# PeterFWS/Structure-PLP-SLAM

Hardware: AMD Instinct MI355X
Metric: frames/sec ORB+LSD extract+match, 640x480 TUM-RGBD, 1/2/4/8 GPU (higher is better)
Workload: dtype u8

## Files before the change

### structure-plp-slam_amd/csrc/line_kernels.hip

```cpp
#include <hip/hip_runtime.h>
#include <stdint.h>

#include <algorithm>
#include <cstdlib>

#include "blur_tile.hpp"
#include "plp_barrier.hpp"
#include "line_device.hpp"
#include "plp_common.hpp"
#include "sincos_ziv.hpp"
#include "xcd_map.hpp"

namespace plp {

struct TileDiv { uint32_t gx_magic, tiles_x_magic; };
static inline TileDiv tile_div(int tiles, int tiles_x, int B) { return TileDiv{plp_div_magic((uint32_t)tiles, (uint64_t)tiles * B), plp_div_magic((uint32_t)tiles_x, (uint64_t)tiles)}; }

__device__ __forceinline__ int reflect101_l(int p, int len) {
    if (len == 1) return 0;
    while (p < 0 || p >= len) p = p < 0 ? -p : 2 * (len - 1) - p;
    return p;
}

__device__ __forceinline__ float fast_atan2_deg_l(float y, float x) {
    const float p1 = 0.9997878412794807f * (float)(180 / 3.14159265358979323846);
    const float p3 = -0.3258083974640975f * (float)(180 / 3.14159265358979323846);
    const float p5 = 0.1555786518463281f * (float)(180 / 3.14159265358979323846);
    const float p7 = -0.04432655554792128f * (float)(180 / 3.14159265358979323846);
    const float eps = (float)2.2204460492503131e-16;
    const float ax = fabsf(x), ay = fabsf(y);
    float a;
    if (ax >= ay) {
        const float c = __fdiv_rn(ay, __fadd_rn(ax, eps));
        const float c2 = __fmul_rn(c, c);
        a = __fmul_rn(__fadd_rn(__fmul_rn(__fadd_rn(__fmul_rn(__fadd_rn(__fmul_rn(p7, c2), p5), c2), p3), c2), p1), c);
    } else {
        const float c = __fdiv_rn(ax, __fadd_rn(ay, eps));
        const float c2 = __fmul_rn(c, c);
        a = __fsub_rn(90.f, __fmul_rn(__fadd_rn(__fmul_rn(__fadd_rn(__fmul_rn(__fadd_rn(__fmul_rn(p7, c2), p5), c2), p3), c2), p1), c));
    }
    if (x < 0) a = __fsub_rn(180.f, a);
    if (y < 0) a = __fsub_rn(360.f, a);
    return a;
}

template <int R>
__global__ __launch_bounds__(256) __attribute__((amdgpu_waves_per_eu(8, 8))) void k_blur_plane(const uint8_t* __restrict__ src, size_t src_fs, int src_pitch,
                                                    uint8_t* __restrict__ dst, size_t dst_fs, int dst_pitch, int w, int h, BlurTapsN taps, TileDiv td) {
    __shared__ BlurTileLds<R> S;
    const int tiles_x = (w + kBlurTW - 1) / kBlurTW;
    unsigned t, f;
    xcd_frame_major(t, f, td.gx_magic);
    const int trow = (int)plp_div(t, (unsigned)tiles_x, td.tiles_x_magic);
    blur_tile<R>(S, src + (size_t)f * src_fs, src_pitch, dst + (size_t)f * dst_fs, dst_pitch, w, h,
                 ((int)t - trow * tiles_x) * kBlurTW, trow * kBlurTH, taps.k);
}

__global__ __launch_bounds__(256) void k_resize_exact(const uint8_t* __restrict__ src, size_t src_fs, int src_pitch,
                                                      uint8_t* __restrict__ dst, size_t dst_fs, int dst_pitch, int dw, int dh,
                                                      ResizeExactTab t) {
    const int dy = blockIdx.y * 4 + threadIdx.y, dx0 = (blockIdx.x * 64 + threadIdx.x) * 4;
    if (dy >= dh || dx0 >= dw) return;
    const uint8_t* s = src + (size_t)blockIdx.z * src_fs;
    const int yo = t.yo[dy], yc = t.yc[dy];
    const uint8_t* S0 = s + (size_t)yo * src_pitch;
    const uint8_t* S1 = yc < 0 ? S0 : S0 + src_pitch;
    const uint32_t b1 = yc < 0 ? 0u : (uint32_t)yc, b0 = 256u - b1;
    uint32_t packed = 0;
#pragma unroll
    for (int i = 0; i < 4; ++i) {
        const int dx = min(dx0 + i, dw - 1);
        const int xo = t.xo[dx], xc = t.xc[dx];
        uint32_t h0, h1;
        if (xc < 0) { h0 = (uint32_t)S0[xo] * 256u; h1 = (uint32_t)S1[xo] * 256u; }
        else {
            h0 = (uint32_t)S0[xo] * (uint32_t)(256 - xc) + (uint32_t)S0[xo + 1] * (uint32_t)xc;
            h1 = (uint32_t)S1[xo] * (uint32_t)(256 - xc) + (uint32_t)S1[xo + 1] * (uint32_t)xc;
        }
        const uint32_t v = (b0 * h0 + b1 * h1 + 32768u) >> 16;
        packed |= min(v, 255u) << (8 * i);
    }
    *reinterpret_cast<uint32_t*>(dst + (size_t)blockIdx.z * dst_fs + (size_t)dy * dst_pitch + dx0) = packed;
}

__global__ __launch_bounds__(256) __attribute__((amdgpu_waves_per_eu(8, 8))) void k_blur_half(const uint8_t* __restrict__ src, size_t src_fs, int src_pitch,
                                                                                           uint8_t* __restrict__ dst, size_t dst_fs, int dst_pitch, int w, int h, BlurTapsN taps, TileDiv td) {
    __shared__ BlurTileLds<5> S;
    const int tiles_x = (w + kBlurTW - 1) / kBlurTW;
    unsigned t, f;
    xcd_frame_major(t, f, td.gx_magic);
    const int trow = (int)plp_div(t, (unsigned)tiles_x, td.tiles_x_magic);
    const int tx0 = ((int)t - trow * tiles_x) * kBlurTW, ty0 = trow * kBlurTH;
    uint8_t* d = dst + (size_t)f * dst_fs;
    blur_tile_core<5>(S, src + (size_t)f * src_fs, src_pitch, w, h, tx0, ty0, taps.k, [&](int r0, int c4, const uint32_t (&rows)[kBlurRS]) {
        const int x = tx0 + c4;
        if (x >= w) return;
#pragma unroll
        for (int j = 0; j < 2; ++j) {
            const int y = ty0 + r0 + 2 * j;
            if (y >= h) continue;
            const uint32_t lo = __builtin_amdgcn_udot4(rows[2 * j], 0x00000101u, __builtin_amdgcn_udot4(rows[2 * j + 1], 0x00000101u, 2u, false), false) >> 2;
            const uint32_t hi = __builtin_amdgcn_udot4(rows[2 * j], 0x01010000u, __builtin_amdgcn_udot4(rows[2 * j + 1], 0x01010000u, 2u, false), false) >> 2;
            *reinterpret_cast<uint16_t*>(d + (size_t)(y >> 1) * dst_pitch + (x >> 1)) = (uint16_t)(lo | (hi << 8));
        }
    });
}

__global__ __launch_bounds__(256) void k_lsd_gradient(LinePlanes P, LsdParams lp) {
    __shared__ uint32_t s_list[256];
    __shared__ uint32_t s_max[4], s_cnt[4];
    const int b = blockIdx.y, tid = threadIdx.x, lane = tid & 63, wv = tid >> 6;
    const int idx = blockIdx.x * 256 + tid;
    const int n = P.sw * P.sh;
    uint32_t g2_def = 0, g2_any = 0, packed = 0;
    if (idx < n) {
        const int y = P.sw_magic ? (int)__umulhi((uint32_t)idx, P.sw_magic) : idx / P.sw, x = idx - y * P.sw;
        if (x < P.sw - 1 && y < P.sh - 1) {
            const uint8_t* s = P.scaled + ((size_t)b * P.sh + y) * P.spitch + x;
            const int DA = (int)s[P.spitch + 1] - (int)s[0];
            const int BC = (int)s[1] - (int)s[P.spitch];
            const int gx = DA + BC, gy = DA - BC;
            const uint32_t g2 = (uint32_t)(gx * gx + gy * gy);
            g2_any = g2;
            if (g2 >= lp.g2_def_min) {
                g2_def = g2;
                packed = (uint32_t)tid | ((uint32_t)(gx + 512) << 8) | ((uint32_t)(gy + 512) << 18);
            }
        }
        P.g2[(size_t)b * n + idx] = lp.seed_exact ? g2_any : g2_def;
    }
    const unsigned long long undef = __ballot(g2_def == 0);
    if (lane == 0 && blockIdx.x * 256 + tid < ((n + 63) / 64) * 64) P.undef[(size_t)b * ((n + 63) / 64) + (blockIdx.x * 256 + tid) / 64] = undef;
    const unsigned long long defm = ~undef;
    const int rank = __popcll(defm & ((1ull << lane) - 1ull));
    uint32_t mx = g2_def;
#pragma unroll
    for (int o = 32; o > 0; o >>= 1) mx = max(mx, (uint32_t)__shfl_xor((int)mx, o));
    if (lane == 0) { s_max[wv] = mx; s_cnt[wv] = (uint32_t)__popcll(defm); }
    wg_barrier();
    const uint32_t c0 = s_cnt[0], c1 = s_cnt[1], c2 = s_cnt[2], c3 = s_cnt[3];
    const int base = (wv > 0 ? (int)c0 : 0) + (wv > 1 ? (int)c1 : 0) + (wv > 2 ? (int)c2 : 0);
    if (g2_def) s_list[base + rank] = packed;
    if (tid == 0) P.blockmax[(size_t)b * gridDim.x + blockIdx.x] = max(max(s_max[0], s_max[1]), max(s_max[2], s_max[3]));
    wg_barrier();
    const int total = (int)(c0 + c1 + c2 + c3);
    if (tid < total) {
        const uint32_t e = s_list[tid];
        const int gx = (int)((e >> 8) & 1023u) - 512, gy = (int)(e >> 18) - 512;
        LsdPix px;
        px.deg = fast_atan2_deg_l((float)gx, (float)-gy);
        px.g2 = (uint32_t)(gx * gx + gy * gy);
        const float fa = (float)((double)px.deg * (3.14159265358979323846 / 180));
        if (!sincos_ziv(fa, &px.cs.x, &px.cs.y)) px.cs = make_float2((float)cos((double)fa), (float)sin((double)fa));
        P.pix[(size_t)b * n + blockIdx.x * 256 + (int)(e & 255u)] = px;
    }
}

__global__ __launch_bounds__(256) void k_lsd_order(LinePlanes P, LsdParams lp, int n_grad_blocks) {
    __shared__ uint32_t cnt[4][1024];
    __shared__ uint32_t s_red[4], s_wsum[4];
    const int b = blockIdx.x, tid = threadIdx.x, lane = tid & 63, q = tid >> 6;
    const int n = P.sw * P.sh, nv = (P.sw - 1) * (P.sh - 1);
    uint32_t mx = 0;
    for (int i = tid; i < n_grad_blocks; i += 256) mx = max(mx, P.blockmax[(size_t)b * n_grad_blocks + i]);
#pragma unroll
    for (int o = 32; o > 0; o >>= 1) mx = max(mx, (uint32_t)__shfl_xor((int)mx, o));
    if (lane == 0) s_red[q] = mx;
    for (int i = tid; i < 4096; i += 256) (&cnt[0][0])[i] = 0;
    wg_barrier();
    mx = max(max(s_red[0], s_red[1]), max(s_red[2], s_red[3]));
    const double max_grad = sqrt((double)mx / 4.0);
    const double bin_coef = (max_grad > 0) ? (double)(lp.n_bins - 1) / max_grad : 0;
    const uint32_t* g2 = P.g2 + (size_t)b * n;
    uint32_t* order = P.order + (size_t)b * nv;
    const int ngroups = (n + 63) / 64, gper = (ngroups + 3) / 4, g0 = q * gper, g1 = min(ngroups, g0 + gper);
    uint32_t* comp = P.reg + (size_t)b * P.reg_frame_stride + (size_t)g0 * 64;
    int ncomp = 0;
    for (int gb = g0; gb < g1; gb += 4) {
        uint32_t v4[4];
#pragma unroll
        for (int u = 0; u < 4; ++u) {
            const int pix = (gb + u) * 64 + lane;
            v4[u] = (gb + u < g1 && pix < n) ? g2[pix] : 0u;
        }
#pragma unroll
        for (int u = 0; u < 4; ++u) {
            const uint32_t v = v4[u];
            const unsigned long long defm = __ballot(v != 0);
            if (!defm) continue;
            if (v) {
                const uint32_t bin = (uint32_t)(int)(sqrt((double)v / 4.0) * bin_coef);
                atomicAdd(&cnt[q][bin], 1u);
                comp[ncomp + __popcll(defm & ((1ull << lane) - 1ull))] = (uint32_t)((gb + u) * 64 + lane) | (bin << kLsdSeedPixBits);
            }
            ncomp += __popcll(defm);
        }
    }
    wg_barrier();
    {
        const int v0 = 1023 - 4 * tid;
        uint32_t c[4][4], tot = 0;
#pragma unroll
        for (int j = 0; j < 4; ++j)
#pragma unroll
            for (int k = 0; k < 4; ++k) { c[j][k] = cnt[k][v0 - j]; tot += c[j][k]; }
        uint32_t inc = tot;
#pragma unroll
        for (int o = 1; o < 64; o <<= 1) { const uint32_t t = (uint32_t)__shfl_up((int)inc, o); if (lane >= o) inc += t; }
        if (lane == 63) s_wsum[q] = inc;
        wg_barrier();
        uint32_t run = inc - tot;
        for (int k = 0; k < q; ++k) run += s_wsum[k];
#pragma unroll
        for (int j = 0; j < 4; ++j)
#pragma unroll
            for (int k = 0; k < 4; ++k) { cnt[k][v0 - j] = run; run += c[j][k]; }
        if (tid == 255) P.n_order[b] = (int32_t)run;
    }
    wg_barrier();
    for (int ib = 0; ib < ncomp; ib += 256) {
    uint32_t e4[4];
#pragma unroll
    for (int u = 0; u < 4; ++u) e4[u] = ib + 64 * u + lane < ncomp ? comp[ib + 64 * u + lane] : 0u;
#pragma unroll
    for (int u = 0; u < 4; ++u) {
        const int i0 = ib + 64 * u;
        if (i0 >= ncomp) break;
        const bool valid = i0 + lane < ncomp;
        const uint32_t e = e4[u];
        const unsigned v = e >> kLsdSeedPixBits;
        unsigned long long peers = __ballot(valid);
#pragma unroll
        for (int bit = 0; bit < 10; ++bit) {
            const unsigned long long m = __ballot((v >> bit) & 1u);
            peers &= ((v >> bit) & 1u) ? m : ~m;
        }
        if (valid) {
// ... 1078 lines not shown
                if (tot <= kMwInline) {
                    if (lane < acc_n) e->inl[lane] = heap_ld(g.reg + lane);
                    else if (lane < tot) e->inl[lane] = g.assumed[lane - acc_n];
                }
                __builtin_amdgcn_fence(__ATOMIC_RELEASE, PLP_MW_SCOPE_NAME);
                __builtin_amdgcn_wave_barrier();
                ++nent; hoff += (tot + 1) & ~1;
                if (lds_ld(&pend_hi[h]) < 0) lds_st(&pend_lo[h], g.my_pos);
                lds_st(&pend_hi[h], g.my_pos);
                lds_st(&buf_n[h * kMwBufs + kbuf], nent);
                mw_forget(g, g.reg, acc_n, 0);
            } else mw_forget(g, g.reg, acc_n, wv);
            __builtin_amdgcn_wave_barrier();
            {
                const int p = (int)mine;
                const int ow = tent_owner(g, p), owh = ow > kMwPending ? ow - kMwPending : ow;
                const bool skip = committed(p) || (ow != 0 && (ow == kMwMainId || owh == wv || cur_pos[min(owh, kMwMaxWaves) - 1] < grp * kMwGroup + lane));
                todo &= __ballot(!skip);
            }
            lds_st(&hstate[h], (grp << 8) | (t + 1));
        }
    }
    if (is_main) {
        if (lane == 0) {
            P.n_raw[b] = min(n_lines, kLineCap);
            int32_t* gs = P.grow_stats + (size_t)b * 4; gs[0] = n_self; gs[1] = n_spec_ok; gs[2] = n_spec_bad; gs[3] = W;
            if (P.prof && b == 0 && prof_on) {
                P.prof[0] = now() - c_begin; P.prof[1] = c_wait; P.prof[2] = c_self;
                P.prof[3] = (long long)hcount[0] | ((long long)hcount[1] << 32); P.prof[4] = n_self; P.prof[5] = (long long)n_spec_ok | ((long long)n_spec_bad << 32);
                P.prof[6] = c_commit; P.prof[7] = c_pub; P.prof[8] = c_grp; P.prof[9] = P.prof[10] = P.prof[11] = 0;
            }
        }
        lds_st(done, 1);
    }
}

__global__ __launch_bounds__(64) void k_keylines(LinePlanes P, LsdParams lp) {
    const int b = blockIdx.x, lane = threadIdx.x;
    const int n = P.n_raw[b];
    const float4* raw = P.raw + (size_t)b * kLineCap;
    plp_keyline* out = P.all_kl + (size_t)b * kLineCap;
    int run = 0;
    for (int base = 0; base < n; base += 64) {
        const int i = base + lane;
        bool keep = false;
        plp_keyline kl{};
        if (i < n) {
            float4 e = raw[i];
            const float fw = (float)P.W, fh = (float)P.H;
            if (e.x < 0) e.x = 0;
            if (e.x >= fw) e.x = fw - 1.0f;
            if (e.z < 0) e.z = 0;
            if (e.z >= fw) e.z = fw - 1.0f;
            if (e.y < 0) e.y = 0;
            if (e.y >= fh) e.y = fh - 1.0f;
            if (e.w < 0) e.w = 0;
            if (e.w >= fh) e.w = fh - 1.0f;
            const double ddx = (double)__fsub_rn(e.x, e.z), ddy = (double)__fsub_rn(e.y, e.w);
            const double length = (double)(float)sqrt(ddx * ddx + ddy * ddy);
            keep = length > (double)lp.min_length;
            kl.startPointX = e.x; kl.startPointY = e.y; kl.endPointX = e.z; kl.endPointY = e.w;
            kl.sPointInOctaveX = e.x; kl.sPointInOctaveY = e.y; kl.ePointInOctaveX = e.z; kl.ePointInOctaveY = e.w;
            kl.lineLength = (float)length;
            const int x1 = __float2int_rn(e.x), y1 = __float2int_rn(e.y), x2 = __float2int_rn(e.z), y2 = __float2int_rn(e.w);
            kl.numOfPixels = max(abs(x2 - x1), abs(y2 - y1)) + 1;
            kl.angle = (float)atan2((double)__fsub_rn(e.w, e.y), (double)__fsub_rn(e.z, e.x));
            kl.octave = 0;
            kl.size = __fmul_rn(__fsub_rn(e.z, e.x), __fsub_rn(e.w, e.y));
            kl.response = __fdiv_rn(kl.lineLength, (float)max(P.W, P.H));
            kl.pt_x = __fdiv_rn(__fadd_rn(e.z, e.x), 2.0f);
            kl.pt_y = __fdiv_rn(__fadd_rn(e.w, e.y), 2.0f);
        }
        const unsigned long long bal = __ballot(keep);
        if (keep) {
            kl.class_id = run + __popcll(bal & ((1ull << lane) - 1ull));
            out[kl.class_id] = kl;
            P.all_kl_dir[(size_t)b * kLineCap + kl.class_id] = make_float2((float)cos((double)kl.angle), (float)sin((double)kl.angle));
        }
        run += __popcll(bal);
    }
    if (lane == 0) P.n_all[b] = run;
}

constexpr int kSobelTW = 120, kSobelTH = 30;
static_assert(sizeof(BlurTileLds<2>::in) >= kBlurTH * (kBlurTW / 4) * 4, "the blurred tile must fit the input rows it replaces");
__global__ __launch_bounds__(256) __attribute__((amdgpu_waves_per_eu(8, 8))) void k_blur_sobel(const uint8_t* __restrict__ src, size_t src_fs, int src_pitch,
                                                                                            short2* __restrict__ dxy, int w, int h, BlurTapsN taps, TileDiv td) {
    __shared__ __attribute__((aligned(16))) BlurTileLds<2> Sb;
    uint32_t* const bt = reinterpret_cast<uint32_t*>(Sb.in);
    const int tiles_x = (w + kSobelTW - 1) / kSobelTW;
    unsigned t, f;
    xcd_frame_major(t, f, td.gx_magic);
    const int trow = (int)plp_div(t, (unsigned)tiles_x, td.tiles_x_magic);
    const int bx0 = ((int)t - trow * tiles_x) * kSobelTW - 4, by0 = trow * kSobelTH - 1;
    blur_tile_core<2>(Sb, src + (size_t)f * src_fs, src_pitch, w, h, bx0, by0, taps.k, [&](int r0, int c4, const uint32_t (&rows)[kBlurRS]) {
#pragma unroll
        for (int rr = 0; rr < kBlurRS; ++rr) bt[(r0 + rr) * (kBlurTW / 4) + c4 / 4] = rows[rr];
    });
    wg_barrier();
    short2* out_frame = dxy + (size_t)f * dxy_frame_entries(w, h);
    const int tiles8 = (w + 7) / 8;
    for (int i = threadIdx.x; i < (kSobelTW / 4) * (kSobelTH / 2); i += 256) {
        const int cgp = i % (kSobelTW / 4), rp = i / (kSobelTW / 4);
        const int x = bx0 + 4 + 4 * cgp, y = by0 + 1 + 2 * rp;
        if (x >= w || y >= h) continue;
        const int cd = 1 + cgp;
        int d[4][4], sm[4][4];
#pragma unroll
        for (int r = 0; r < 4; ++r) {
            const uint32_t* q = &bt[(2 * rp + r) * (kBlurTW / 4) + cd];
            const uint32_t A = q[-1], Bv = q[0], Cv = q[1];
            const int p[6] = {(int)(A >> 24), (int)(Bv & 255u), (int)((Bv >> 8) & 255u), (int)((Bv >> 16) & 255u), (int)(Bv >> 24), (int)(Cv & 255u)};
#pragma unroll
            for (int k = 0; k < 4; ++k) { d[r][k] = p[k + 2] - p[k]; sm[r][k] = p[k] + 2 * p[k + 1] + p[k + 2]; }
        }
#pragma unroll
        for (int j = 0; j < 2; ++j) {
            if (y + j >= h) continue;
            uint32_t out[4];
#pragma unroll
            for (int k = 0; k < 4; ++k)
                out[k] = ((uint32_t)(d[j][k] + 2 * d[j + 1][k] + d[j + 2][k]) & 0xffffu) | ((uint32_t)(sm[j + 2][k] - sm[j][k]) << 16);
            *reinterpret_cast<uint4*>(out_frame + dxy_index(x, y + j, tiles8)) = make_uint4(out[0], out[1], out[2], out[3]);
        }
    }
}

__constant__ int c_comb[32][2] = {{0, 1}, {0, 2}, {0, 3}, {0, 4}, {0, 5}, {0, 6}, {1, 2}, {1, 3}, {1, 4}, {1, 5}, {1, 6},
                                  {2, 3}, {2, 4}, {2, 5}, {2, 6}, {2, 7}, {2, 8}, {3, 4}, {3, 5}, {3, 6}, {3, 7}, {3, 8},
                                  {4, 5}, {4, 6}, {4, 7}, {4, 8}, {5, 6}, {5, 7}, {5, 8}, {6, 7}, {6, 8}, {7, 8}};

constexpr int kLbdU = 8;
__global__ __launch_bounds__(256) void k_lbd(LinePlanes P, LbdWeightsDev W) {
    __shared__ float s_row[4][63][8];
    __shared__ float s_des[4][72], s_des2[4][72], s_norm[4][4];
    const int lane = threadIdx.x & 63, wv = __builtin_amdgcn_readfirstlane((int)(threadIdx.x >> 6)), b = blockIdx.y;
    const int n_lines = P.n_all[b];
    for (int li = blockIdx.x * 4 + wv; li < n_lines; li += gridDim.x * 4) {
    const plp_keyline kl = P.all_kl[(size_t)b * kLineCap + li];
    const short2* dxyImg = P.dxy + (size_t)b * dxy_frame_entries(P.W, P.H);
    const int tiles8 = (P.W + 7) / 8;
    const short imageWidth = (short)(P.W - 1), imageHeight = (short)(P.H - 1);
    const short lengthOfLSP = (short)kl.numOfPixels;
    const short halfWidth = (short)((lengthOfLSP - 1) / 2), halfHeight = 31;
    const float midX = (float)(0.5 * (double)__fadd_rn(kl.sPointInOctaveX, kl.ePointInOctaveX));
    const float midY = (float)(0.5 * (double)__fadd_rn(kl.sPointInOctaveY, kl.ePointInOctaveY));
    const float2 dir = P.all_kl_dir[(size_t)b * kLineCap + li];
    const float dL0 = dir.x, dL1 = dir.y;
    const float dO0 = -dL1, dO1 = dL0;
    if (lane < 63) {
        float sCorX0 = __fadd_rn(__fadd_rn(__fmul_rn(-dL0, (float)halfWidth), __fmul_rn(dL1, (float)halfHeight)), midX);
        float sCorY0 = __fadd_rn(__fsub_rn(__fmul_rn(-dL1, (float)halfWidth), __fmul_rn(dL0, (float)halfHeight)), midY);
        for (int r = 0; r < lane; ++r) { sCorX0 = __fsub_rn(sCorX0, dL1); sCorY0 = __fadd_rn(sCorY0, dL0); }
        float sCorX = sCorX0, sCorY = sCorY0;
        float pgdL = 0, ngdL = 0, pgdO = 0, ngdO = 0;
        for (int w0 = 0; w0 < lengthOfLSP; w0 += kLbdU) {
            int off[kLbdU];
#pragma unroll
            for (int u = 0; u < kLbdU; ++u) {
                short t = (short)roundf(sCorX);
                const short xCor = (t < 0) ? 0 : (t > imageWidth) ? imageWidth : t;
                t = (short)roundf(sCorY);
                const short yCor = (t < 0) ? 0 : (t > imageHeight) ? imageHeight : t;
                off[u] = dxy_index(xCor, yCor, tiles8);
                sCorX = __fadd_rn(sCorX, dL0);
                sCorY = __fadd_rn(sCorY, dL1);
            }
            short2 vxy[kLbdU];
#pragma unroll
            for (int u = 0; u < kLbdU; ++u) vxy[u] = dxyImg[off[u]];
#pragma unroll
            for (int u = 0; u < kLbdU; ++u) {
                if (w0 + u < lengthOfLSP) {
                    const float fx = (float)vxy[u].x, fy = (float)vxy[u].y;
                    const float gDL = __fadd_rn(__fmul_rn(fx, dL0), __fmul_rn(fy, dL1));
                    const float gDO = __fadd_rn(__fmul_rn(fx, dO0), __fmul_rn(fy, dO1));
                    if (gDL > 0) pgdL = __fadd_rn(pgdL, gDL); else ngdL = __fsub_rn(ngdL, gDL);
                    if (gDO > 0) pgdO = __fadd_rn(pgdO, gDO); else ngdO = __fsub_rn(ngdO, gDO);
                }
            }
        }
        const float cg = W.g[lane];
        pgdL = __fmul_rn(cg, pgdL); ngdL = __fmul_rn(cg, ngdL); pgdO = __fmul_rn(cg, pgdO); ngdO = __fmul_rn(cg, ngdO);
        float* r = s_row[wv][lane];
        r[0] = pgdL; r[1] = ngdL; r[2] = __fmul_rn(pgdL, pgdL); r[3] = __fmul_rn(ngdL, ngdL);
        r[4] = pgdO; r[5] = ngdO; r[6] = __fmul_rn(pgdO, pgdO); r[7] = __fmul_rn(ngdO, ngdO);
    }
    __builtin_amdgcn_fence(__ATOMIC_RELEASE, "workgroup");
    __builtin_amdgcn_wave_barrier();
    for (int item = lane; item < 72; item += 64) {
        const int band = item >> 3, comp = item & 7;
        const bool sq = (comp == 2 || comp == 3 || comp == 6 || comp == 7);
        float acc = 0;
        for (int hID = max(0, (band - 1) * 7); hID < min(63, (band + 2) * 7); ++hID) {
            const int rb = hID / 7;
            const float c = rb == band ? W.l[hID % 7 + 7] : (rb == band + 1 ? W.l[hID % 7 + 14] : W.l[hID % 7]);
            const float v = s_row[wv][hID][comp];
            acc = sq ? __fadd_rn(acc, __fmul_rn(__fmul_rn(c, c), v)) : __fadd_rn(acc, __fmul_rn(c, v));
        }
        s_des[wv][item] = acc;
    }
    __builtin_amdgcn_fence(__ATOMIC_RELEASE, "workgroup");
    __builtin_amdgcn_wave_barrier();
    float* des = s_des2[wv];
    auto wave_sync = [] { __builtin_amdgcn_fence(__ATOMIC_ACQ_REL, "workgroup"); __builtin_amdgcn_wave_barrier(); };
    if (lane < 36) {
        const int band = lane >> 2, k = lane & 3;
        const float invN = (band == 0 || band == 8) ? (float)(1.0 / (7 * 2.0)) : (float)(1.0 / (7 * 3.0));
        const float* sb = &s_des[wv][band * 8];
        const int mi = (k < 2) ? k : k + 2, qi = mi + 2;
        const float temp = __fmul_rn(sb[mi], invN);
        des[band * 8 + k] = temp;
        des[band * 8 + 4 + k] = sqrtf(__fsub_rn(__fmul_rn(sb[qi], invN), __fmul_rn(temp, temp)));
    }
    wave_sync();
    if (lane == 0) {
        float tempM = 0, tempS = 0;
        for (int band = 0; band < 9; ++band) {
            const float* v = des + 8 * band;
            for (int k = 0; k < 4; ++k) tempM = __fadd_rn(tempM, __fmul_rn(v[k], v[k]));
            for (int k = 4; k < 8; ++k) tempS = __fadd_rn(tempS, __fmul_rn(v[k], v[k]));
        }
        s_norm[wv][0] = __fdiv_rn(1.0f, sqrtf(tempM));
        s_norm[wv][1] = __fdiv_rn(1.0f, sqrtf(tempS));
    }
    wave_sync();
    for (int i = lane; i < 72; i += 64) {
        float v = __fmul_rn(des[i], s_norm[wv][(i >> 2) & 1]);
        if ((double)v > 0.4) v = (float)0.4;
        des[i] = v;
    }
    wave_sync();
    if (lane == 0) {
        float temp = 0;
        for (int i = 0; i < 72; ++i) temp = __fadd_rn(temp, __fmul_rn(des[i], des[i]));
        s_norm[wv][2] = __fdiv_rn(1.0f, sqrtf(temp));
    }
    wave_sync();
    for (int i = lane; i < 72; i += 64) des[i] = __fmul_rn(des[i], s_norm[wv][2]);
    wave_sync();
    if (lane < 32) {
        const float* f1 = des + 8 * c_comb[lane][0];
        const float* f2 = des + 8 * c_comb[lane][1];
        unsigned r = 0;
        for (int i = 0; i < 8; ++i) r += (f1[i] > f2[i]) ? (1u << i) : 0u;
        P.all_lbd[((size_t)b * kLineCap + li) * 32 + lane] = (uint8_t)r;
    }
    __builtin_amdgcn_fence(__ATOMIC_ACQ_REL, "workgroup");
    __builtin_amdgcn_wave_barrier();
    }
}

__global__ __launch_bounds__(64) void k_line_finalize(LinePlanes P, LsdParams lp, plp_keyline* __restrict__ out_kl,
                                                      uint8_t* __restrict__ out_lbd, double* __restrict__ out_fn, int cap,
                                                      int32_t* __restrict__ out_counts) {
    const int b = blockIdx.x, lane = threadIdx.x;
    const int n = P.n_all[b];
    int run = 0;
    for (int base = 0; base < n; base += 64) {
        const int i = base + lane;
        plp_keyline kl{};
        bool keep = false;
        if (i < n) { kl = P.all_kl[(size_t)b * kLineCap + i]; keep = kl.octave == 0 && kl.lineLength >= lp.keep_length; }
        const unsigned long long bal = __ballot(keep);
        const int o = run + __popcll(bal & ((1ull << lane) - 1ull));
        if (keep && o < cap) {
            out_kl[(size_t)b * cap + o] = kl;
            const uint4* s = reinterpret_cast<const uint4*>(P.all_lbd + ((size_t)b * kLineCap + i) * 32);
            uint4* d = reinterpret_cast<uint4*>(out_lbd + ((size_t)b * cap + o) * 32);
            d[0] = s[0]; d[1] = s[1];
            const double sx = kl.startPointX, sy = kl.startPointY, ex = kl.endPointX, ey = kl.endPointY;
            const double a = sy * 1.0 - 1.0 * ey, bb = 1.0 * ex - sx * 1.0, c = sx * ey - sy * ex;
            const double nrm = sqrt(a * a + bb * bb);
            double* f = out_fn + ((size_t)b * cap + o) * 3;
            f[0] = a / nrm; f[1] = bb / nrm; f[2] = c / nrm;
        }
        run += __popcll(bal);
    }
    if (lane == 0) {
        out_counts[b] = min(run, cap);
        if (run > cap) atomicOr(P.status, 1);
    }
}

void launch_line_front(hipStream_t st, const LinePlanes& P, const LsdParams& lp, const ResizeExactTab& rt, const BlurTapsN& t11,
                       const BlurTapsN& t5, const LbdWeightsDev& w, plp_keyline* out_kl, uint8_t* out_lbd, double* out_fn, int cap,
                       int32_t* out_counts, int B, hipEvent_t* ev, int grow_waves, const SeedSortBufs* seed_exact, bool mw_ok) {
    auto mark = [&](int i) { if (ev) (void)hipEventRecord(ev[i], st); };
    const bool sobel_first = !ev;
    const size_t plane_fs = (size_t)P.pitch * P.H, splane_fs = (size_t)P.spitch * P.sh;
    const int tiles = ((P.W + 127) / 128) * ((P.H + kBlurTH - 1) / kBlurTH);
    const int sobel_tiles = ((P.W + kSobelTW - 1) / kSobelTW) * ((P.H + kSobelTH - 1) / kSobelTH);
    const TileDiv blur_td = tile_div(tiles, (P.W + 127) / 128, B), sobel_td = tile_div(sobel_tiles, (P.W + kSobelTW - 1) / kSobelTW, B);
    mark(0);
    if (sobel_first) hipLaunchKernelGGL(k_blur_sobel, dim3(sobel_tiles, B), dim3(256), 0, st, P.img, P.img_frame_stride, P.img_pitch, P.dxy, P.W, P.H, t5, sobel_td);
    if (P.half_exact)
        hipLaunchKernelGGL(k_blur_half, dim3(tiles, B), dim3(256), 0, st, P.img, P.img_frame_stride, P.img_pitch, P.scaled, splane_fs, P.spitch, P.W, P.H, t11, blur_td);
    else {
        hipLaunchKernelGGL(k_blur_plane<5>, dim3(tiles, B), dim3(256), 0, st, P.img, P.img_frame_stride, P.img_pitch, P.blur11, plane_fs,
                           P.pitch, P.W, P.H, t11, blur_td);
        hipLaunchKernelGGL(k_resize_exact, dim3((P.sw + 255) / 256, (P.sh + 3) / 4, B), dim3(64, 4), 0, st, P.blur11, plane_fs, P.pitch,
                           P.scaled, splane_fs, P.spitch, P.sw, P.sh, rt);
    }
    mark(1);
    const int n = P.sw * P.sh;
    hipLaunchKernelGGL(k_lsd_gradient, dim3((n + 255) / 256, B), dim3(256), 0, st, P, lp);
    mark(2);
    if (seed_exact) launch_seed_order_exact(st, P, lp, B, seed_exact->ent, seed_exact->ws, seed_exact->ws_stride);
    else hipLaunchKernelGGL(k_lsd_order, dim3(B), dim3(256), 0, st, P, lp, (n + 255) / 256);
    mark(3);
    constexpr int ring = 256;
    const size_t per_wave = (size_t)((((n + 31) / 32 + 1) & ~1) + ring) * 4;
    const int wpb = (int)std::max<size_t>(1, std::min<size_t>(4, 65536 / per_wave));
    MwLayout L{};
    size_t mw_bytes = 0;
    const int want_waves = grow_waves > 0 ? std::min(grow_waves, kMwMaxWaves) : kMwMaxWaves;
    if (mw_ok && B <= kLsdMwMaxFrames && want_waves >= 2 && P.mw_heap && P.reg_frame_stride >= 2 * (size_t)n) {
        const int nw_al = (((n + 31) / 32 + 1) & ~1), groups_cap = ((P.sw - 1) * (P.sh - 1) + kMwGroup - 1) / kMwGroup + 64 / kMwGroup;
        for (int w = want_waves; w >= 2; --w) {
            const size_t bytes = (size_t)5 * nw_al * 4 + (size_t)w * (nw_al + 256 + kMwAssumed + 2) * 4 + (8 + (4 + 2 * kMwBufs) * kMwMaxWaves) * 4 + ((groups_cap + 15) & ~15) + 16 +
                                 (size_t)(w - 1) * kMwBufs * kMwEntries * sizeof(MwEntry);
            if (bytes <= 160 * 1024) { L.waves = w; L.ring = 256; L.nw_al = nw_al; L.n_groups_cap = groups_cap; L.lookahead = kMwBufs * (w - 1); L.policy = 0; L.prof = ev ? 1 : 0; mw_bytes = bytes; break; }
        }
    }
    if (L.waves >= 2)
        hipLaunchKernelGGL(k_lsd_grow_mw, dim3(B), dim3(64 * L.waves), mw_bytes, st, P, lp, L);
    else
        hipLaunchKernelGGL(k_lsd_grow, dim3((B + wpb - 1) / wpb), dim3(64 * wpb), per_wave * wpb, st, P, lp, B, wpb, ring);
    mark(4);
    hipLaunchKernelGGL(k_keylines, dim3(B), dim3(64), 0, st, P, lp);
    mark(5);
    if (!sobel_first) hipLaunchKernelGGL(k_blur_sobel, dim3(sobel_tiles, B), dim3(256), 0, st, P.img, P.img_frame_stride, P.img_pitch, P.dxy, P.W, P.H, t5, sobel_td);
    mark(6);
    const int lbd_blocks = B >= 64 ? 2 : 16;
    hipLaunchKernelGGL(k_lbd, dim3(lbd_blocks, B), dim3(256), 0, st, P, w);
    mark(7);
    hipLaunchKernelGGL(k_line_finalize, dim3(B), dim3(64), 0, st, P, lp, out_kl, out_lbd, out_fn, cap, out_counts);
    mark(8);
}

hipError_t grow_configure() {
    return hipFuncSetAttribute(reinterpret_cast<const void*>(k_lsd_grow), hipFuncAttributeMaxDynamicSharedMemorySize, (int)kLsdGrowLdsBytes);
}
hipError_t grow_mw_configure() {
    return hipFuncSetAttribute(reinterpret_cast<const void*>(k_lsd_grow_mw), hipFuncAttributeMaxDynamicSharedMemorySize, (int)(160 * 1024));
}

}
```

Measured before the change: 92960.

## Replace LDS-tiled blurs with per-wave register strip blurs using DPP halos

Adds a BlurStrip helper in which each wavefront slides vertically down a column strip. It keeps the separable Gaussian's row sums in registers, gets horizontal halo pixels from neighbour lanes through DPP, and uses udot2/udot4 for the filter taps. k_blur_half and k_blur_sobel are rebuilt on it, dropping LDS tiles and workgroup barriers, and both get template edge and non-edge paths. k_lsd_gradient now has each wave handle its own 256-pixel block with per-wave compaction lists, so block max and compaction need fewer barriers. The new paths raise register pressure and carry complex border-reflection logic, which risks correctness at image edges.

```diff
diff --git a/structure-plp-slam_amd/csrc/blur_strip.hpp b/structure-plp-slam_amd/csrc/blur_strip.hpp
--- /dev/null
+++ b/structure-plp-slam_amd/csrc/blur_strip.hpp
@@ -0,0 +1,131 @@
+#pragma once
+#include <hip/hip_runtime.h>
+#include <stdint.h>
+
+namespace plp {
+
+typedef unsigned short bs_us2 __attribute__((ext_vector_type(2)));
+__device__ __forceinline__ uint32_t bs_dot2(uint32_t a, uint32_t b, uint32_t c) {
+    return __builtin_amdgcn_udot2(__builtin_bit_cast(bs_us2, a), __builtin_bit_cast(bs_us2, b), c, false);
+}
+__device__ __forceinline__ uint32_t bs_from_left(uint32_t v) { return (uint32_t)__builtin_amdgcn_update_dpp(0, (int)v, 0x138, 0xf, 0xf, false); }
+__device__ __forceinline__ uint32_t bs_from_right(uint32_t v) { return (uint32_t)__builtin_amdgcn_update_dpp(0, (int)v, 0x130, 0xf, 0xf, false); }
+__device__ __forceinline__ uint32_t bs_load_u32_any(const uint8_t* p) {
+    uint32_t v;
+    __builtin_memcpy(&v, p, 4);
+    return v;
+}
+
+template <int R> struct BlurStrip {
+    static_assert(R >= 1 && R <= 8, "two halo lanes at most");
+    static constexpr int K = 2 * R + 1, NP = R + 1;
+    static constexpr int HL = (R + 3) / 4;
+    static constexpr int kW = 4 * (64 - 2 * HL);
+    static constexpr int kSteps = NP % 2 ? 2 * NP : NP;
+    static constexpr int kTripRows = 2 * kSteps;
+    static constexpr int ND = 2 * HL + 1, OFF = 4 * HL - R, TM = (K + 3 + 3) / 4;
+
+    static __device__ __forceinline__ int lane_x(int x0) { return x0 + 4 * ((int)(threadIdx.x & 63) - HL); }
+    static __device__ __forceinline__ bool touches_border(int x0, int w) { return x0 == 0 || x0 + kW + 4 * HL > w; }
+
+    template <bool EDGE, class Emit>
+    static __device__ __forceinline__ void run(const uint8_t* __restrict__ src, int sp, int w, int h, int x, int ya, int yb, const int* __restrict__ k, Emit emit) {
+        uint32_t tp[4][TM];
+#pragma unroll
+        for (int e = 0; e < 4; ++e)
+#pragma unroll
+            for (int m = 0; m < TM; ++m) {
+                uint32_t v = 0;
+#pragma unroll
+                for (int b = 0; b < 4; ++b) {
+                    const int i = 4 * m + b - e;
+                    if (i >= 0 && i < K) v |= (uint32_t)k[i] << (8 * b);
+                }
+                tp[e][m] = v;
+            }
+        uint32_t te[NP], to[NP];
+#pragma unroll
+        for (int j = 0; j < NP; ++j) {
+            te[j] = (uint32_t)k[2 * j] | (2 * j + 1 < K ? (uint32_t)k[2 * j + 1] << 16 : 0u);
+            to[j] = (j > 0 ? (uint32_t)k[2 * j - 1] : 0u) | ((uint32_t)k[2 * j] << 16);
+        }
+        uint32_t a_own = (uint32_t)x, a_mir = 0, sel = 0x03020100u;
+        if (EDGE) {
+            const int n = w - x;
+            a_own = (uint32_t)min(max(x, 0), (w - 1) & ~3);
+            const int m = x < 0 ? -x - 3 : n <= 0 ? 2 * (w - 1) - x - 3 : n < 4 ? w - 5 : x;
+            a_mir = (uint32_t)min(max(m, 0), w - 4);
+            sel = x < 0 || n <= 0 ? 0x04050607u : n == 1 ? 0x05060700u : n == 2 ? 0x06070100u : n == 3 ? 0x07020100u : 0x03020100u;
+        }
+        struct Raw { uint32_t own, mir; };
+        auto load_row = [&](int y) -> Raw {
+            int yy = y < 0 ? -y : y >= h ? 2 * (h - 1) - y : y;
+            yy = min(max(yy, 0), h - 1);
+            const uint8_t* row = src + (uint32_t)(yy * sp);
+            Raw q;
+            q.own = *reinterpret_cast<const uint32_t*>(row + a_own);
+            q.mir = EDGE ? bs_load_u32_any(row + a_mir) : 0u;
+            return q;
+        };
+        auto hsum = [&](const Raw& q, uint32_t (&a)[4]) {
+            uint32_t d[ND];
+            d[HL] = EDGE ? __builtin_amdgcn_perm(q.mir, q.own, sel) : q.own;
+#pragma unroll
+            for (int i = 0; i < HL; ++i) { d[HL - 1 - i] = bs_from_left(d[HL - i]); d[HL + 1 + i] = bs_from_right(d[HL + i]); }
+#pragma unroll
+            for (int o = 0; o < 4; ++o) {
+                const int s = OFF + o, q0 = s >> 2, e = s & 3;
+                uint32_t acc = 0;
+#pragma unroll
+                for (int m = 0; m < (e + K + 3) / 4; ++m) acc = __builtin_amdgcn_udot4(d[q0 + m], tp[e][m], acc, false);
+                a[o] = acc;
+            }
+        };
+        auto pair = [&](const Raw& ra, const Raw& rb, uint32_t (&p)[4]) {
+            uint32_t ha[4], hb[4];
+            hsum(ra, ha);
+            hsum(rb, hb);
+#pragma unroll
+            for (int o = 0; o < 4; ++o) p[o] = ha[o] | (hb[o] << 16);
+        };
+
+        uint32_t P[NP][4];
+        Raw Q[4];
+        {
+            Raw c[2 * (NP - 1)];
+#pragma unroll
+            for (int i = 0; i < 2 * (NP - 1); ++i) c[i] = load_row(ya - R + i);
+#pragma unroll
+            for (int i = 0; i < 4; ++i) Q[i] = load_row(ya + R + i);
+#pragma unroll
+            for (int j = 0; j < NP - 1; ++j) pair(c[2 * j], c[2 * j + 1], P[j]);
+        }
+        for (int r0 = ya; r0 < yb; r0 += kTripRows) {
+#pragma unroll
+            for (int s = 0; s < kSteps; ++s) {
+                const int r = r0 + 2 * s;
+                Raw* q = &Q[2 * (s & 1)];
+                const Raw ra = q[0], rb = q[1];
+                q[0] = load_row(r + R + 4); q[1] = load_row(r + R + 5);
+                pair(ra, rb, P[NP - 1]);
+                uint32_t ev[4], od[4];
+#pragma unroll
+                for (int o = 0; o < 4; ++o) {
+                    uint32_t a = 32768u, b = 32768u;
+#pragma unroll
+                    for (int j = 0; j < NP; ++j) { a = bs_dot2(P[j][o], te[j], a); b = bs_dot2(P[j][o], to[j], b); }
+                    ev[o] = a; od[o] = b;
+                }
+                const uint32_t oe = __builtin_amdgcn_perm(ev[1], ev[0], 0x0c0c0602u) | __builtin_amdgcn_perm(ev[3], ev[2], 0x06020c0cu);
+                const uint32_t oo = __builtin_amdgcn_perm(od[1], od[0], 0x0c0c0602u) | __builtin_amdgcn_perm(od[3], od[2], 0x06020c0cu);
+                emit(r, oe, oo);
+#pragma unroll
+                for (int j = 0; j < NP - 1; ++j)
+#pragma unroll
+                    for (int o = 0; o < 4; ++o) P[j][o] = P[j + 1][o];
+            }
+        }
+    }
+};
+
+}
diff --git a/structure-plp-slam_amd/csrc/line_kernels.hip b/structure-plp-slam_amd/csrc/line_kernels.hip
--- a/structure-plp-slam_amd/csrc/line_kernels.hip
+++ b/structure-plp-slam_amd/csrc/line_kernels.hip
@@ -4,6 +4,7 @@
 #include <algorithm>
 #include <cstdlib>
 
+#include "blur_strip.hpp"
 #include "blur_tile.hpp"
 #include "plp_barrier.hpp"
 #include "line_device.hpp"
@@ -83,76 +84,89 @@
     *reinterpret_cast<uint32_t*>(dst + (size_t)blockIdx.z * dst_fs + (size_t)dy * dst_pitch + dx0) = packed;
 }
 
-__global__ __launch_bounds__(256) __attribute__((amdgpu_waves_per_eu(8, 8))) void k_blur_half(const uint8_t* __restrict__ src, size_t src_fs, int src_pitch,
-                                                                                           uint8_t* __restrict__ dst, size_t dst_fs, int dst_pitch, int w, int h, BlurTapsN taps, TileDiv td) {
-    __shared__ BlurTileLds<5> S;
-    const int tiles_x = (w + kBlurTW - 1) / kBlurTW;
-    unsigned t, f;
-    xcd_frame_major(t, f, td.gx_magic);
-    const int trow = (int)plp_div(t, (unsigned)tiles_x, td.tiles_x_magic);
-    const int tx0 = ((int)t - trow * tiles_x) * kBlurTW, ty0 = trow * kBlurTH;
-    uint8_t* d = dst + (size_t)f * dst_fs;
-    blur_tile_core<5>(S, src + (size_t)f * src_fs, src_pitch, w, h, tx0, ty0, taps.k, [&](int r0, int c4, const uint32_t (&rows)[kBlurRS]) {
-        const int x = tx0 + c4;
-        if (x >= w) return;
-#pragma unroll
-        for (int j = 0; j < 2; ++j) {
-            const int y = ty0 + r0 + 2 * j;
-            if (y >= h) continue;
-            const uint32_t lo = __builtin_amdgcn_udot4(rows[2 * j], 0x00000101u, __builtin_amdgcn_udot4(rows[2 * j + 1], 0x00000101u, 2u, false), false) >> 2;
-            const uint32_t hi = __builtin_amdgcn_udot4(rows[2 * j], 0x01010000u, __builtin_amdgcn_udot4(rows[2 * j + 1], 0x01010000u, 2u, false), false) >> 2;
-            *reinterpret_cast<uint16_t*>(d + (size_t)(y >> 1) * dst_pitch + (x >> 1)) = (uint16_t)(lo | (hi << 8));
-        }
+constexpr int kHalfW = BlurStrip<5>::kW, kHalfH = 8 * BlurStrip<5>::kTripRows;
+template <bool EDGE>
+__device__ __forceinline__ void blur_half_strip(const uint8_t* __restrict__ src, int sp, uint8_t* __restrict__ dst, int dp, int w, int h, int x, int y0, int y1,
+                                                const int* __restrict__ k) {
+    const int lane = threadIdx.x & 63;
+    const bool out_lane = lane >= BlurStrip<5>::HL && lane <= 63 - BlurStrip<5>::HL && x < w;
+    BlurStrip<5>::run<EDGE>(src, sp, w, h, x, y0, y1, k, [&](int r, uint32_t even, uint32_t odd) {
+        const uint32_t lo = __builtin_amdgcn_udot4(even, 0x00000101u, __builtin_amdgcn_udot4(odd, 0x00000101u, 2u, false), false) >> 2;
+        const uint32_t hi = __builtin_amdgcn_udot4(even, 0x01010000u, __builtin_amdgcn_udot4(odd, 0x01010000u, 2u, false), false) >> 2;
+        if (out_lane && r < y1) *reinterpret_cast<uint16_t*>(dst + (uint32_t)(__mul24(r >> 1, dp) + (x >> 1))) = (uint16_t)(lo | (hi << 8));
     });
 }
 
-__global__ __launch_bounds__(256) void k_lsd_gradient(LinePlanes P, LsdParams lp) {
-    __shared__ uint32_t s_list[256];
-    __shared__ uint32_t s_max[4], s_cnt[4];
-    const int b = blockIdx.y, tid = threadIdx.x, lane = tid & 63, wv = tid >> 6;
-    const int idx = blockIdx.x * 256 + tid;
-    const int n = P.sw * P.sh;
-    uint32_t g2_def = 0, g2_any = 0, packed = 0;
-    if (idx < n) {
+__global__ __launch_bounds__(256) void k_blur_half(const uint8_t* __restrict__ src, size_t src_fs, int src_pitch, uint8_t* __restrict__ dst, size_t dst_fs, int dst_pitch,
+                                                   int w, int h, BlurTapsN taps, TileDiv td, int n_strips) {
+    unsigned ub, f;
+    xcd_frame_major(ub, f, td.gx_magic);
+    const int t = (int)ub * 4 + __builtin_amdgcn_readfirstlane((int)(threadIdx.x >> 6));
+    if (t >= n_strips) return;
+    const int strips_x = (w + kHalfW - 1) / kHalfW;
+    const int srow = (int)plp_div((unsigned)t, (unsigned)strips_x, td.tiles_x_magic);
+    const int x0 = (t - srow * strips_x) * kHalfW, x = BlurStrip<5>::lane_x(x0);
+    const int y0 = srow * kHalfH, y1 = min(y0 + kHalfH, h);
+    if (BlurStrip<5>::touches_border(x0, w))
+        blur_half_strip<true>(src + (size_t)f * src_fs, src_pitch, dst + (size_t)f * dst_fs, dst_pitch, w, h, x, y0, y1, taps.k);
+    else
+        blur_half_strip<false>(src + (size_t)f * src_fs, src_pitch, dst + (size_t)f * dst_fs, dst_pitch, w, h, x, y0, y1, taps.k);
+}
+
+constexpr int kGradBlock = 256;
+__global__ __launch_bounds__(256) void k_lsd_gradient(LinePlanes P, LsdParams lp, int n_blocks) {
+    __shared__ uint32_t s_list[4][kGradBlock];
+    __shared__ uint32_t s_cnt[4];
+    const int b = blockIdx.y, tid = threadIdx.x, lane = tid & 63, wv = __builtin_amdgcn_readfirstlane(tid >> 6);
+    const int blk = (int)blockIdx.x * 4 + wv;
+    const int n = P.sw * P.sh, base = blk * kGradBlock;
+    const uint8_t* frame = P.scaled + (size_t)b * P.sh * P.spitch;
+    bool live[4];
+    uint8_t px00[4], px01[4], px10[4], px11[4];
+#pragma unroll
+    for (int j = 0; j < 4; ++j) {
+        const int idx = base + 64 * j + lane;
         const int y = P.sw_magic ? (int)__umulhi((uint32_t)idx, P.sw_magic) : idx / P.sw, x = idx - y * P.sw;
-        if (x < P.sw - 1 && y < P.sh - 1) {
-            const uint8_t* s = P.scaled + ((size_t)b * P.sh + y) * P.spitch + x;
-            const int DA = (int)s[P.spitch + 1] - (int)s[0];
-            const int BC = (int)s[1] - (int)s[P.spitch];
-            const int gx = DA + BC, gy = DA - BC;
-            const uint32_t g2 = (uint32_t)(gx * gx + gy * gy);
-            g2_any = g2;
-            if (g2 >= lp.g2_def_min) {
-                g2_def = g2;
-                packed = (uint32_t)tid | ((uint32_t)(gx + 512) << 8) | ((uint32_t)(gy + 512) << 18);
-            }
-        }
-        P.g2[(size_t)b * n + idx] = lp.seed_exact ? g2_any : g2_def;
-    }
-    const unsigned long long undef = __ballot(g2_def == 0);
-    if (lane == 0 && blockIdx.x * 256 + tid < ((n + 63) / 64) * 64) P.undef[(size_t)b * ((n + 63) / 64) + (blockIdx.x * 256 + tid) / 64] = undef;
-    const unsigned long long defm = ~undef;
-    const int rank = __popcll(defm & ((1ull << lane) - 1ull));
-    uint32_t mx = g2_def;
+        live[j] = idx < n && x < P.sw - 1 && y < P.sh - 1;
+        const uint8_t* s = frame + (live[j] ? (uint32_t)(y * P.spitch + x) : 0u);
+        px00[j] = s[0]; px01[j] = s[1]; px10[j] = s[P.spitch]; px11[j] = s[P.spitch + 1];
+    }
+    uint32_t mx = 0;
+    int total = 0;
+#pragma unroll
+    for (int j = 0; j < 4; ++j) {
+        const int idx = base + 64 * j + lane;
+        const int DA = (int)px11[j] - (int)px00[j];
+        const int BC = (int)px01[j] - (int)px10[j];
+        const int gx = DA + BC, gy = DA - BC;
+        const uint32_t g2_any = live[j] ? (uint32_t)(gx * gx + gy * gy) : 0u;
+        const uint32_t g2_def = g2_any >= lp.g2_def_min ? g2_any : 0u;
+        if (idx < n) P.g2[(size_t)b * n + idx] = lp.seed_exact ? g2_any : g2_def;
+        const unsigned long long undef = __ballot(g2_def == 0);
+        if (lane == 0 && base + 64 * j < ((n + 63) / 64) * 64) P.undef[(size_t)b * ((n + 63) / 64) + (base + 64 * j) / 64] = undef;
+        const unsigned long long defm = ~undef;
+        if (g2_def) s_list[wv][total + __popcll(defm & ((1ull << lane) - 1ull))] = (uint32_t)(64 * j + lane) | ((uint32_t)(gx + 512) << 8) | ((uint32_t)(gy + 512) << 18);
+        total += __popcll(defm);
+        mx = max(mx, g2_def);
+    }
 #pragma unroll
     for (int o = 32; o > 0; o >>= 1) mx = max(mx, (uint32_t)__shfl_xor((int)mx, o));
-    if (lane == 0) { s_max[wv] = mx; s_cnt[wv] = (uint32_t)__popcll(defm); }
+    if (lane == 0) {
+        s_cnt[wv] = (uint32_t)total;
+        if (blk < n_blocks) P.blockmax[(size_t)b * n_blocks + blk] = mx;
+    }
     wg_barrier();
-    const uint32_t c0 = s_cnt[0], c1 = s_cnt[1], c2 = s_cnt[2], c3 = s_cnt[3];
-    const int base = (wv > 0 ? (int)c0 : 0) + (wv > 1 ? (int)c1 : 0) + (wv > 2 ? (int)c2 : 0);
-    if (g2_def) s_list[base + rank] = packed;
-    if (tid == 0) P.blockmax[(size_t)b * gridDim.x + blockIdx.x] = max(max(s_max[0], s_max[1]), max(s_max[2], s_max[3]));
-    wg_barrier();
-    const int total = (int)(c0 + c1 + c2 + c3);
-    if (tid < total) {
-        const uint32_t e = s_list[tid];
+    const int c0 = (int)s_cnt[0], c1 = c0 + (int)s_cnt[1], c2 = c1 + (int)s_cnt[2], c3 = c2 + (int)s_cnt[3];
+    for (int g = tid; g < c3; g += 256) {
+        const int seg = (g >= c0) + (g >= c1) + (g >= c2);
+        const uint32_t e = s_list[seg][g - (seg == 0 ? 0 : seg == 1 ? c0 : seg == 2 ? c1 : c2)];
         const int gx = (int)((e >> 8) & 1023u) - 512, gy = (int)(e >> 18) - 512;
         LsdPix px;
         px.deg = fast_atan2_deg_l((float)gx, (float)-gy);
         px.g2 = (uint32_t)(gx * gx + gy * gy);
         const float fa = (float)((double)px.deg * (3.14159265358979323846 / 180));
         if (!sincos_ziv(fa, &px.cs.x, &px.cs.y)) px.cs = make_float2((float)cos((double)fa), (float)sin((double)fa));
-        P.pix[(size_t)b * n + blockIdx.x * 256 + (int)(e & 255u)] = px;
+        P.pix[(size_t)b * n + ((int)blockIdx.x * 4 + seg) * kGradBlock + (int)(e & 255u)] = px;
     }
 }
 
@@ -1397,48 +1411,57 @@
     if (lane == 0) P.n_all[b] = run;
 }
 
-constexpr int kSobelTW = 120, kSobelTH = 30;
-static_assert(sizeof(BlurTileLds<2>::in) >= kBlurTH * (kBlurTW / 4) * 4, "the blurred tile must fit the input rows it replaces");
-__global__ __launch_bounds__(256) __attribute__((amdgpu_waves_per_eu(8, 8))) void k_blur_sobel(const uint8_t* __restrict__ src, size_t src_fs, int src_pitch,
-                                                                                            short2* __restrict__ dxy, int w, int h, BlurTapsN taps, TileDiv td) {
-    __shared__ __attribute__((aligned(16))) BlurTileLds<2> Sb;
-    uint32_t* const bt = reinterpret_cast<uint32_t*>(Sb.in);
-    const int tiles_x = (w + kSobelTW - 1) / kSobelTW;
-    unsigned t, f;
-    xcd_frame_major(t, f, td.gx_magic);
-    const int trow = (int)plp_div(t, (unsigned)tiles_x, td.tiles_x_magic);
-    const int bx0 = ((int)t - trow * tiles_x) * kSobelTW - 4, by0 = trow * kSobelTH - 1;
-    blur_tile_core<2>(Sb, src + (size_t)f * src_fs, src_pitch, w, h, bx0, by0, taps.k, [&](int r0, int c4, const uint32_t (&rows)[kBlurRS]) {
-#pragma unroll
-        for (int rr = 0; rr < kBlurRS; ++rr) bt[(r0 + rr) * (kBlurTW / 4) + c4 / 4] = rows[rr];
+constexpr int kSobelW = BlurStrip<2>::kW, kSobelH = 6 * BlurStrip<2>::kTripRows - 2;
+template <bool EDGE>
+__device__ __forceinline__ void blur_sobel_strip(const uint8_t* __restrict__ src, int sp, short2* __restrict__ out_frame, int w, int h, int x, int y0, int y1,
+                                                 const int* __restrict__ k) {
+    const int lane = threadIdx.x & 63, tiles8 = (w + 7) / 8;
+    const bool out_lane = lane >= 1 && lane <= 62 && x < w;
+    uint32_t sel_lo = 0x06050403u, sel_hi = 0x04030201u;
+    if (EDGE) {
+        const int n = w - x;
+        sel_lo = x == 0 ? 0x06050405u : n == 1 ? 0x06030403u : n == 2 ? 0x04050403u : sel_lo;
+        sel_hi = n == 3 ? 0x04010201u : n == 4 ? 0x02030201u : sel_hi;
+    }
+    auto row = [&](uint32_t own, int (&d)[4], int (&sm)[4]) {
+        const uint32_t lo = __builtin_amdgcn_perm(own, bs_from_left(own), sel_lo), hi = __builtin_amdgcn_perm(bs_from_right(own), own, sel_hi);
+        const int p[6] = {(int)(lo & 255u), (int)((lo >> 8) & 255u), (int)((lo >> 16) & 255u), (int)(lo >> 24), (int)((hi >> 16) & 255u), (int)(hi >> 24)};
+#pragma unroll
+        for (int c = 0; c < 4; ++c) { d[c] = p[c + 2] - p[c]; sm[c] = p[c] + 2 * p[c + 1] + p[c + 2]; }
+    };
+    auto store = [&](int y, const int (&da)[4], const int (&db)[4], const int (&dc)[4], const int (&sa)[4], const int (&sc)[4]) {
+        uint32_t out[4];
+#pragma unroll
+        for (int c = 0; c < 4; ++c) out[c] = ((uint32_t)(da[c] + 2 * db[c] + dc[c]) & 0xffffu) | ((uint32_t)(sc[c] - sa[c]) << 16);
+        if (out_lane && y >= y0 && y < y1) *reinterpret_cast<uint4*>(out_frame + dxy_index(x, y, tiles8)) = make_uint4(out[0], out[1], out[2], out[3]);
+    };
+    int d1[4] = {}, s1[4] = {}, d2[4] = {}, s2[4] = {};
+    BlurStrip<2>::run<EDGE>(src, sp, w, h, x, y0 - 1, y1 + 1, k, [&](int r, uint32_t even, uint32_t odd) {
+        int d3[4], s3[4], d4[4], s4[4];
+        row(even, d3, s3);
+        row(odd, d4, s4);
+        store(r - 1, d1, d2, d3, s1, s3);
+        store(r, d2, d3, d4, s2, s4);
+#pragma unroll
+        for (int c = 0; c < 4; ++c) { d1[c] = d3[c]; s1[c] = s3[c]; d2[c] = d4[c]; s2[c] = s4[c]; }
     });
-    wg_barrier();
+}
+
+__global__ __launch_bounds__(256) void k_blur_sobel(const uint8_t* __restrict__ src, size_t src_fs, int src_pitch, short2* __restrict__ dxy, int w, int h, BlurTapsN taps,
+                                                    TileDiv td, int n_strips) {
+    unsigned ub, f;
+    xcd_frame_major(ub, f, td.gx_magic);
+    const int t = (int)ub * 4 + __builtin_amdgcn_readfirstlane((int)(threadIdx.x >> 6));
+    if (t >= n_strips) return;
+    const int strips_x = (w + kSobelW - 1) / kSobelW;
+    const int srow = (int)plp_div((unsigned)t, (unsigned)strips_x, td.tiles_x_magic);
+    const int x0 = (t - srow * strips_x) * kSobelW, x = BlurStrip<2>::lane_x(x0);
+    const int y0 = srow * kSobelH, y1 = min(y0 + kSobelH, h);
     short2* out_frame = dxy + (size_t)f * dxy_frame_entries(w, h);
-    const int tiles8 = (w + 7) / 8;
-    for (int i = threadIdx.x; i < (kSobelTW / 4) * (kSobelTH / 2); i += 256) {
-        const int cgp = i % (kSobelTW / 4), rp = i / (kSobelTW / 4);
-        const int x = bx0 + 4 + 4 * cgp, y = by0 + 1 + 2 * rp;
-        if (x >= w || y >= h) continue;
-        const int cd = 1 + cgp;
-        int d[4][4], sm[4][4];
-#pragma unroll
-        for (int r = 0; r < 4; ++r) {
-            const uint32_t* q = &bt[(2 * rp + r) * (kBlurTW / 4) + cd];
-            const uint32_t A = q[-1], Bv = q[0], Cv = q[1];
-            const int p[6] = {(int)(A >> 24), (int)(Bv & 255u), (int)((Bv >> 8) & 255u), (int)((Bv >> 16) & 255u), (int)(Bv >> 24), (int)(Cv & 255u)};
-#pragma unroll
-            for (int k = 0; k < 4; ++k) { d[r][k] = p[k + 2] - p[k]; sm[r][k] = p[k] + 2 * p[k + 1] + p[k + 2]; }
-        }
-#pragma unroll
-        for (int j = 0; j < 2; ++j) {
-            if (y + j >= h) continue;
-            uint32_t out[4];
-#pragma unroll
-            for (int k = 0; k < 4; ++k)
-                out[k] = ((uint32_t)(d[j][k] + 2 * d[j + 1][k] + d[j + 2][k]) & 0xffffu) | ((uint32_t)(sm[j + 2][k] - sm[j][k]) << 16);
-            *reinterpret_cast<uint4*>(out_frame + dxy_index(x, y + j, tiles8)) = make_uint4(out[0], out[1], out[2], out[3]);
-        }
-    }
+    if (BlurStrip<2>::touches_border(x0, w))
+        blur_sobel_strip<true>(src + (size_t)f * src_fs, src_pitch, out_frame, w, h, x, y0, y1, taps.k);
+    else
+        blur_sobel_strip<false>(src + (size_t)f * src_fs, src_pitch, out_frame, w, h, x, y0, y1, taps.k);
 }
 
 __constant__ int c_comb[32][2] = {{0, 1}, {0, 2}, {0, 3}, {0, 4}, {0, 5}, {0, 6}, {1, 2}, {1, 3}, {1, 4}, {1, 5}, {1, 6},
@@ -1605,12 +1628,15 @@
     const bool sobel_first = !ev;
     const size_t plane_fs = (size_t)P.pitch * P.H, splane_fs = (size_t)P.spitch * P.sh;
     const int tiles = ((P.W + 127) / 128) * ((P.H + kBlurTH - 1) / kBlurTH);
-    const int sobel_tiles = ((P.W + kSobelTW - 1) / kSobelTW) * ((P.H + kSobelTH - 1) / kSobelTH);
-    const TileDiv blur_td = tile_div(tiles, (P.W + 127) / 128, B), sobel_td = tile_div(sobel_tiles, (P.W + kSobelTW - 1) / kSobelTW, B);
+    const TileDiv blur_td = tile_div(tiles, (P.W + 127) / 128, B);
+    auto strip_div = [&](int strips, int strips_x) { return TileDiv{plp_div_magic((uint32_t)((strips + 3) / 4), (uint64_t)((strips + 3) / 4) * B), plp_div_magic((uint32_t)strips_x, (uint64_t)strips + 3)}; };
+    const int half_sx = (P.W + kHalfW - 1) / kHalfW, half_strips = half_sx * ((P.H + kHalfH - 1) / kHalfH);
+    const int sobel_sx = (P.W + kSobelW - 1) / kSobelW, sobel_strips = sobel_sx * ((P.H + kSobelH - 1) / kSobelH);
+    const TileDiv half_td = strip_div(half_strips, half_sx), sobel_td = strip_div(sobel_strips, sobel_sx);
     mark(0);
-    if (sobel_first) hipLaunchKernelGGL(k_blur_sobel, dim3(sobel_tiles, B), dim3(256), 0, st, P.img, P.img_frame_stride, P.img_pitch, P.dxy, P.W, P.H, t5, sobel_td);
+    if (sobel_first) hipLaunchKernelGGL(k_blur_sobel, dim3((sobel_strips + 3) / 4, B), dim3(256), 0, st, P.img, P.img_frame_stride, P.img_pitch, P.dxy, P.W, P.H, t5, sobel_td, sobel_strips);
     if (P.half_exact)
-        hipLaunchKernelGGL(k_blur_half, dim3(tiles, B), dim3(256), 0, st, P.img, P.img_frame_stride, P.img_pitch, P.scaled, splane_fs, P.spitch, P.W, P.H, t11, blur_td);
+        hipLaunchKernelGGL(k_blur_half, dim3((half_strips + 3) / 4, B), dim3(256), 0, st, P.img, P.img_frame_stride, P.img_pitch, P.scaled, splane_fs, P.spitch, P.W, P.H, t11, half_td, half_strips);
     else {
         hipLaunchKernelGGL(k_blur_plane<5>, dim3(tiles, B), dim3(256), 0, st, P.img, P.img_frame_stride, P.img_pitch, P.blur11, plane_fs,
                            P.pitch, P.W, P.H, t11, blur_td);
@@ -1618,11 +1644,11 @@
                            P.scaled, splane_fs, P.spitch, P.sw, P.sh, rt);
     }
     mark(1);
-    const int n = P.sw * P.sh;
-    hipLaunchKernelGGL(k_lsd_gradient, dim3((n + 255) / 256, B), dim3(256), 0, st, P, lp);
+    const int n = P.sw * P.sh, n_grad_blocks = (n + kGradBlock - 1) / kGradBlock;
+    hipLaunchKernelGGL(k_lsd_gradient, dim3((n_grad_blocks + 3) / 4, B), dim3(256), 0, st, P, lp, n_grad_blocks);
     mark(2);
     if (seed_exact) launch_seed_order_exact(st, P, lp, B, seed_exact->ent, seed_exact->ws, seed_exact->ws_stride);
-    else hipLaunchKernelGGL(k_lsd_order, dim3(B), dim3(256), 0, st, P, lp, (n + 255) / 256);
+    else hipLaunchKernelGGL(k_lsd_order, dim3(B), dim3(256), 0, st, P, lp, n_grad_blocks);
     mark(3);
     constexpr int ring = 256;
     const size_t per_wave = (size_t)((((n + 31) / 32 + 1) & ~1) + ring) * 4;
@@ -1645,7 +1671,7 @@
     mark(4);
     hipLaunchKernelGGL(k_keylines, dim3(B), dim3(64), 0, st, P, lp);
     mark(5);
-    if (!sobel_first) hipLaunchKernelGGL(k_blur_sobel, dim3(sobel_tiles, B), dim3(256), 0, st, P.img, P.img_frame_stride, P.img_pitch, P.dxy, P.W, P.H, t5, sobel_td);
+    if (!sobel_first) hipLaunchKernelGGL(k_blur_sobel, dim3((sobel_strips + 3) / 4, B), dim3(256), 0, st, P.img, P.img_frame_stride, P.img_pitch, P.dxy, P.W, P.H, t5, sobel_td, sobel_strips);
     mark(6);
     const int lbd_blocks = B >= 64 ? 2 : 16;
     hipLaunchKernelGGL(k_lbd, dim3(lbd_blocks, B), dim3(256), 0, st, P, w);
```

Result: no change. 93330 (median of 4 runs) (+0.4%).
